# KikeM/romtime

Hardware: AMD Instinct MI355X
Metric: snapshot-DoF/s for POD build (higher is better)
Workload: dtype f64

## Files before the change

romtime_amd/csrc/tallskinny.hip:

```cpp
#include "common.h"

typedef double d2 __attribute__((ext_vector_type(2)));
typedef double d4 __attribute__((ext_vector_type(4)));

namespace {

constexpr int TS_THREADS = 256;
constexpr int TS_KS = 32;
constexpr int TS_SA = 34;

struct TsParams {
  const double* X;
  const double* T;
  double* Y;
  long N, ldx, ldt, ldy;
  int n, k;
};

template <int NT, int RB>
__global__ __launch_bounds__(TS_THREADS, RB == 2 ? (NT <= 4 ? 3 : 1) : (NT <= 4 ? 4 : 2)) void tallskinny_kernel(const TsParams p) {
  constexpr int TS_BM = 64 * RB;
  constexpr int TS_XL = TS_BM * TS_KS / 2 / TS_THREADS;
  constexpr int KP = 16 * NT;
  constexpr int TL = (TS_KS * KP / 2 + TS_THREADS - 1) / TS_THREADS;
  __shared__ __attribute__((aligned(16))) double sA[TS_BM * TS_SA];
  __shared__ __attribute__((aligned(16))) double sT[TS_KS * KP];
  const int tid = threadIdx.x, lane = tid & 63, l15 = lane & 15, l4 = lane >> 4;
  const int wid = __builtin_amdgcn_readfirstlane(tid >> 6);
  const long row0 = (long)blockIdx.x * TS_BM;
  const bool xvec = ((p.ldx & 1) == 0) && ((reinterpret_cast<size_t>(p.X) & 15) == 0);
  const bool tvec = ((p.ldt & 1) == 0) && ((reinterpret_cast<size_t>(p.T) & 15) == 0);

  d4 acc[RB][NT];
#pragma unroll
  for (int b = 0; b < RB; ++b)
#pragma unroll
    for (int j = 0; j < NT; ++j) acc[b][j] = d4{0.0, 0.0, 0.0, 0.0};

  d2 xr[TS_XL], tr[TL];
  auto fetch = [&](int c0) {
#pragma unroll
    for (int i = 0; i < TS_XL; ++i) {
      const int q = tid + TS_THREADS * i, r = q / (TS_KS / 2), c = c0 + 2 * (q % (TS_KS / 2));
      const long row = row0 + r;
      d2 v{0.0, 0.0};
      if (row < p.N) {
        const double* src = p.X + row * p.ldx + c;
        if (xvec && c + 1 < p.n) {
          v = *reinterpret_cast<const d2*>(src);
        } else {
          if (c < p.n) v.x = src[0];
          if (c + 1 < p.n) v.y = src[1];
        }
      }
      xr[i] = v;
    }
#pragma unroll
    for (int i = 0; i < TL; ++i) {
      const int q = tid + TS_THREADS * i, kk = q / (KP / 2), j = 2 * (q % (KP / 2));
      d2 v{0.0, 0.0};
      if (kk < TS_KS && c0 + kk < p.n) {
        const double* src = p.T + (long)(c0 + kk) * p.ldt + j;
        if (tvec && j + 1 < p.k) {
          v = *reinterpret_cast<const d2*>(src);
        } else {
          if (j < p.k) v.x = src[0];
          if (j + 1 < p.k) v.y = src[1];
        }
      }
      tr[i] = v;
    }
  };
  auto commit = [&]() {
#pragma unroll
    for (int i = 0; i < TS_XL; ++i) {
      const int q = tid + TS_THREADS * i, r = q / (TS_KS / 2), c = 2 * (q % (TS_KS / 2));
      *reinterpret_cast<d2*>(&sA[r * TS_SA + c]) = xr[i];
    }
#pragma unroll
    for (int i = 0; i < TL; ++i) {
      const int q = tid + TS_THREADS * i, kk = q / (KP / 2), j = 2 * (q % (KP / 2));
      if (kk < TS_KS) *reinterpret_cast<d2*>(&sT[kk * KP + j]) = tr[i];
    }
  };

  fetch(0);
  commit();
  __syncthreads();
  const double* fa = sA + (16 * wid + l15) * TS_SA + l4;
  const double* fb = sT + l4 * KP + l15;
  int c0 = 0;
  const bool fast = xvec && tvec && (row0 + TS_BM <= p.N) && (p.n % TS_KS == 0) && ((p.k & 1) == 0) &&
                    ((long)TS_BM * p.ldx * 8 < (1L << 31)) && ((long)TS_KS * p.ldt * 8 < (1L << 31));
  if (fast) {
    const char* gx = reinterpret_cast<const char*>(p.X + row0 * p.ldx + TS_KS);
    const char* gt = reinterpret_cast<const char*>(p.T + (long)TS_KS * p.ldt);
    const unsigned xoff = (unsigned)(((long)(tid / (TS_KS / 2)) * p.ldx + 2 * (tid % (TS_KS / 2))) * 8);
    const long xstep = (long)(TS_THREADS / (TS_KS / 2)) * p.ldx * 8;
    unsigned toff[TL];
    bool tuse[TL];
#pragma unroll
    for (int i = 0; i < TL; ++i) {
      const int q = tid + TS_THREADS * i, kk = q / (KP / 2), j = 2 * (q % (KP / 2));
      toff[i] = (unsigned)(((long)kk * p.ldt + j) * 8);
      tuse[i] = j + 1 < p.k;
      tr[i] = d2{0.0, 0.0};
    }
    const long tstage = (long)TS_KS * p.ldt * 8;
    for (; c0 + TS_KS < p.n; c0 += TS_KS) {
#pragma unroll
      for (int i = 0; i < TS_XL; ++i) xr[i] = *reinterpret_cast<const d2*>(gx + i * xstep + xoff);
#pragma unroll
      for (int i = 0; i < TL; ++i)
        if (tuse[i]) tr[i] = *reinterpret_cast<const d2*>(gt + toff[i]);
#pragma unroll
      for (int k4 = 0; k4 < TS_KS / 4; ++k4) {
        double bq[NT];
#pragma unroll
        for (int j = 0; j < NT; ++j) bq[j] = fb[4 * k4 * KP + 16 * j];
#pragma unroll
        for (int b = 0; b < RB; ++b) {
          const double a = fa[64 * b * TS_SA + 4 * k4];
#pragma unroll
          for (int j = 0; j < NT; ++j) acc[b][j] = __builtin_amdgcn_mfma_f64_16x16x4f64(a, bq[j], acc[b][j], 0, 0, 0);
        }
      }
      gx += TS_KS * 8;
      gt += tstage;
      __syncthreads();
      commit();
      __syncthreads();
    }
  }
  for (; c0 < p.n; c0 += TS_KS) {
    const bool more = c0 + TS_KS < p.n;
    if (more) fetch(c0 + TS_KS);
#pragma unroll
    for (int k4 = 0; k4 < TS_KS / 4; ++k4) {
      double bq[NT];
#pragma unroll
      for (int j = 0; j < NT; ++j) bq[j] = fb[4 * k4 * KP + 16 * j];
#pragma unroll
      for (int b = 0; b < RB; ++b) {
        const double a = fa[64 * b * TS_SA + 4 * k4];
#pragma unroll
        for (int j = 0; j < NT; ++j) acc[b][j] = __builtin_amdgcn_mfma_f64_16x16x4f64(a, bq[j], acc[b][j], 0, 0, 0);
      }
    }
    __syncthreads();
    if (more) commit();
    __syncthreads();
  }
#pragma unroll
  for (int b = 0; b < RB; ++b)
#pragma unroll
    for (int j = 0; j < NT; ++j)
#pragma unroll
      for (int c = 0; c < 4; ++c) {
        const long row = row0 + 64 * b + 16 * wid + l4 + 4 * c;
        const int col = 16 * j + l15;
        if (row < p.N && col < p.k) p.Y[row * p.ldy + col] = acc[b][j][c];
      }
}

}

int rt_tallskinny(rt_ctx* ctx, const double* X, int64_t ldx, const double* T, int64_t ldt, int64_t N, int64_t n,
                  int64_t k, double* Y, int64_t ldy) {
  if (k > 128 || n < 2 * TS_KS || N < 64L * ctx->num_cus) return RT_ERR_UNSUPPORTED;
  TsParams p{X, T, Y, (long)N, (long)ldx, (long)ldt, (long)ldy, (int)n, (int)k};
  const int nt = (int)((k + 15) / 16);
  const int rb = (nt <= 4 && N >= 128L * 4 * ctx->num_cus) ? 2 : 1;
  const int bm = 64 * rb;
  const unsigned grid = (unsigned)((N + bm - 1) / bm);
  if (ctx->profile) {
    if (!ctx->ev0) {
      RT_HIP_CHECK(ctx, hipEventCreate(&ctx->ev0));
      RT_HIP_CHECK(ctx, hipEventCreate(&ctx->ev1));
    }
    RT_HIP_CHECK(ctx, hipEventRecord(ctx->ev0, ctx->stream));
  }
#define TS_LAUNCH(NT_)                                                                                                  \
  if (rb == 2) hipLaunchKernelGGL((tallskinny_kernel<(NT_ <= 4 ? NT_ : 4), 2>), dim3(grid), dim3(TS_THREADS), 0, ctx->stream, p); \
  else hipLaunchKernelGGL((tallskinny_kernel<NT_, 1>), dim3(grid), dim3(TS_THREADS), 0, ctx->stream, p)
  switch (nt) {
    case 1: TS_LAUNCH(1); break;
    case 2: TS_LAUNCH(2); break;
    case 3: TS_LAUNCH(3); break;
    case 4: TS_LAUNCH(4); break;
    case 5: TS_LAUNCH(5); break;
    case 6: TS_LAUNCH(6); break;
    case 7: TS_LAUNCH(7); break;
    default: TS_LAUNCH(8); break;
  }
#undef TS_LAUNCH
  RT_HIP_CHECK(ctx, hipGetLastError());
  if (ctx->profile) {
    RT_HIP_CHECK(ctx, hipEventRecord(ctx->ev1, ctx->stream));
    ctx->ev_valid = true;
  }
  ctx->last_grid = grid; ctx->last_splits = 1; ctx->last_tile = bm * 1000 + 16 * nt;
  return RT_OK;
}
```

Before: 90.20 billion.

## Handle ragged k tail with 4x4x4 f64 MFMA instead of padding to 16

When k is not a multiple of 16, the last column group is computed with 4x4x4 f64 MFMA blocks, 4 columns each, instead of a full 16x16x4 tile. This cuts wasted matrix-core work and T loads on padded columns. Templates now split into full tiles (KF) and narrow groups (G), and the dispatch switch picks among many more instantiations. The narrow MFMA layout adds risk in how lanes map to output rows and columns, and small tails use a different instruction mix.

```diff
diff --git a/romtime_amd/csrc/tallskinny.hip b/romtime_amd/csrc/tallskinny.hip
--- a/romtime_amd/csrc/tallskinny.hip
+++ b/romtime_amd/csrc/tallskinny.hip
@@ -17,12 +17,15 @@
   int n, k;
 };
 
-template <int NT, int RB>
-__global__ __launch_bounds__(TS_THREADS, RB == 2 ? (NT <= 4 ? 3 : 1) : (NT <= 4 ? 4 : 2)) void tallskinny_kernel(const TsParams p) {
+template <int KF, int G, int RB>
+__global__ __launch_bounds__(TS_THREADS, RB == 2 ? (KF + (G > 0) <= 4 ? 3 : 1) : (KF + (G > 0) <= 4 ? 4 : 2)) void tallskinny_kernel(const TsParams p) {
+  constexpr int NT = KF + (G > 0);
   constexpr int TS_BM = 64 * RB;
   constexpr int TS_XL = TS_BM * TS_KS / 2 / TS_THREADS;
   constexpr int KP = 16 * NT;
-  constexpr int TL = (TS_KS * KP / 2 + TS_THREADS - 1) / TS_THREADS;
+  constexpr int KW = 16 * KF + 4 * G;
+  constexpr int TL = (TS_KS * KW / 2 + TS_THREADS - 1) / TS_THREADS;
+  constexpr int KF1 = KF > 0 ? KF : 1, G1 = G > 0 ? G : 1;
   __shared__ __attribute__((aligned(16))) double sA[TS_BM * TS_SA];
   __shared__ __attribute__((aligned(16))) double sT[TS_KS * KP];
   const int tid = threadIdx.x, lane = tid & 63, l15 = lane & 15, l4 = lane >> 4;
@@ -31,11 +34,15 @@
   const bool xvec = ((p.ldx & 1) == 0) && ((reinterpret_cast<size_t>(p.X) & 15) == 0);
   const bool tvec = ((p.ldt & 1) == 0) && ((reinterpret_cast<size_t>(p.T) & 15) == 0);
 
-  d4 acc[RB][NT];
-#pragma unroll
-  for (int b = 0; b < RB; ++b)
-#pragma unroll
-    for (int j = 0; j < NT; ++j) acc[b][j] = d4{0.0, 0.0, 0.0, 0.0};
+  d4 acc[RB][KF1];
+  double accg[RB][G1];
+#pragma unroll
+  for (int b = 0; b < RB; ++b) {
+#pragma unroll
+    for (int j = 0; j < KF1; ++j) acc[b][j] = d4{0.0, 0.0, 0.0, 0.0};
+#pragma unroll
+    for (int g = 0; g < G1; ++g) accg[b][g] = 0.0;
+  }
 
   d2 xr[TS_XL], tr[TL];
   auto fetch = [&](int c0) {
@@ -57,7 +64,7 @@
     }
 #pragma unroll
     for (int i = 0; i < TL; ++i) {
-      const int q = tid + TS_THREADS * i, kk = q / (KP / 2), j = 2 * (q % (KP / 2));
+      const int q = tid + TS_THREADS * i, kk = q / (KW / 2), j = 2 * (q % (KW / 2));
       d2 v{0.0, 0.0};
       if (kk < TS_KS && c0 + kk < p.n) {
         const double* src = p.T + (long)(c0 + kk) * p.ldt + j;
@@ -79,7 +86,7 @@
     }
 #pragma unroll
     for (int i = 0; i < TL; ++i) {
-      const int q = tid + TS_THREADS * i, kk = q / (KP / 2), j = 2 * (q % (KP / 2));
+      const int q = tid + TS_THREADS * i, kk = q / (KW / 2), j = 2 * (q % (KW / 2));
       if (kk < TS_KS) *reinterpret_cast<d2*>(&sT[kk * KP + j]) = tr[i];
     }
   };
@@ -89,6 +96,25 @@
   __syncthreads();
   const double* fa = sA + (16 * wid + l15) * TS_SA + l4;
   const double* fb = sT + l4 * KP + l15;
+  const double* fg = sT + l4 * KP + 16 * KF + (lane & 3);
+  auto multiply = [&]() {
+#pragma unroll
+    for (int k4 = 0; k4 < TS_KS / 4; ++k4) {
+      double bq[KF1], bg[G1];
+#pragma unroll
+      for (int j = 0; j < KF; ++j) bq[j] = fb[4 * k4 * KP + 16 * j];
+#pragma unroll
+      for (int g = 0; g < G; ++g) bg[g] = fg[4 * k4 * KP + 4 * g];
+#pragma unroll
+      for (int b = 0; b < RB; ++b) {
+        const double a = fa[64 * b * TS_SA + 4 * k4];
+#pragma unroll
+        for (int j = 0; j < KF; ++j) acc[b][j] = __builtin_amdgcn_mfma_f64_16x16x4f64(a, bq[j], acc[b][j], 0, 0, 0);
+#pragma unroll
+        for (int g = 0; g < G; ++g) accg[b][g] = __builtin_amdgcn_mfma_f64_4x4x4f64(a, bg[g], accg[b][g], 0, 0, 0);
+      }
+    }
+  };
   int c0 = 0;
   const bool fast = xvec && tvec && (row0 + TS_BM <= p.N) && (p.n % TS_KS == 0) && ((p.k & 1) == 0) &&
                     ((long)TS_BM * p.ldx * 8 < (1L << 31)) && ((long)TS_KS * p.ldt * 8 < (1L << 31));
@@ -101,9 +127,9 @@
     bool tuse[TL];
 #pragma unroll
     for (int i = 0; i < TL; ++i) {
-      const int q = tid + TS_THREADS * i, kk = q / (KP / 2), j = 2 * (q % (KP / 2));
+      const int q = tid + TS_THREADS * i, kk = q / (KW / 2), j = 2 * (q % (KW / 2));
       toff[i] = (unsigned)(((long)kk * p.ldt + j) * 8);
-      tuse[i] = j + 1 < p.k;
+      tuse[i] = kk < TS_KS && j + 1 < p.k;
       tr[i] = d2{0.0, 0.0};
     }
     const long tstage = (long)TS_KS * p.ldt * 8;
@@ -113,18 +139,7 @@
 #pragma unroll
       for (int i = 0; i < TL; ++i)
         if (tuse[i]) tr[i] = *reinterpret_cast<const d2*>(gt + toff[i]);
-#pragma unroll
-      for (int k4 = 0; k4 < TS_KS / 4; ++k4) {
-        double bq[NT];
-#pragma unroll
-        for (int j = 0; j < NT; ++j) bq[j] = fb[4 * k4 * KP + 16 * j];
-#pragma unroll
-        for (int b = 0; b < RB; ++b) {
-          const double a = fa[64 * b * TS_SA + 4 * k4];
-#pragma unroll
-          for (int j = 0; j < NT; ++j) acc[b][j] = __builtin_amdgcn_mfma_f64_16x16x4f64(a, bq[j], acc[b][j], 0, 0, 0);
-        }
-      }
+      multiply();
       gx += TS_KS * 8;
       gt += tstage;
       __syncthreads();
@@ -135,32 +150,39 @@
   for (; c0 < p.n; c0 += TS_KS) {
     const bool more = c0 + TS_KS < p.n;
     if (more) fetch(c0 + TS_KS);
-#pragma unroll
-    for (int k4 = 0; k4 < TS_KS / 4; ++k4) {
-      double bq[NT];
-#pragma unroll
-      for (int j = 0; j < NT; ++j) bq[j] = fb[4 * k4 * KP + 16 * j];
-#pragma unroll
-      for (int b = 0; b < RB; ++b) {
-        const double a = fa[64 * b * TS_SA + 4 * k4];
-#pragma unroll
-        for (int j = 0; j < NT; ++j) acc[b][j] = __builtin_amdgcn_mfma_f64_16x16x4f64(a, bq[j], acc[b][j], 0, 0, 0);
-      }
-    }
+    multiply();
     __syncthreads();
     if (more) commit();
     __syncthreads();
   }
 #pragma unroll
-  for (int b = 0; b < RB; ++b)
-#pragma unroll
-    for (int j = 0; j < NT; ++j)
+  for (int b = 0; b < RB; ++b) {
+#pragma unroll
+    for (int j = 0; j < KF; ++j)
 #pragma unroll
       for (int c = 0; c < 4; ++c) {
         const long row = row0 + 64 * b + 16 * wid + l4 + 4 * c;
         const int col = 16 * j + l15;
         if (row < p.N && col < p.k) p.Y[row * p.ldy + col] = acc[b][j][c];
       }
+#pragma unroll
+    for (int g = 0; g < G; ++g) {
+      const long row = row0 + 64 * b + 16 * wid + (l15 & 12) + l4;
+      const int col = 16 * KF + 4 * g + (lane & 3);
+      if (row < p.N && col < p.k) p.Y[row * p.ldy + col] = accg[b][g];
+    }
+  }
+}
+
+template <int KF, int G>
+void ts_launch(int rb, unsigned grid, hipStream_t stream, const TsParams& p) {
+  if constexpr (KF + (G > 0) <= 4) {
+    if (rb == 2) {
+      hipLaunchKernelGGL((tallskinny_kernel<KF, G, 2>), dim3(grid), dim3(TS_THREADS), 0, stream, p);
+      return;
+    }
+  }
+  hipLaunchKernelGGL((tallskinny_kernel<KF, G, 1>), dim3(grid), dim3(TS_THREADS), 0, stream, p);
 }
 
 }
@@ -180,20 +202,17 @@
     }
     RT_HIP_CHECK(ctx, hipEventRecord(ctx->ev0, ctx->stream));
   }
-#define TS_LAUNCH(NT_)                                                                                                  \
-  if (rb == 2) hipLaunchKernelGGL((tallskinny_kernel<(NT_ <= 4 ? NT_ : 4), 2>), dim3(grid), dim3(TS_THREADS), 0, ctx->stream, p); \
-  else hipLaunchKernelGGL((tallskinny_kernel<NT_, 1>), dim3(grid), dim3(TS_THREADS), 0, ctx->stream, p)
-  switch (nt) {
-    case 1: TS_LAUNCH(1); break;
-    case 2: TS_LAUNCH(2); break;
-    case 3: TS_LAUNCH(3); break;
-    case 4: TS_LAUNCH(4); break;
-    case 5: TS_LAUNCH(5); break;
-    case 6: TS_LAUNCH(6); break;
-    case 7: TS_LAUNCH(7); break;
-    default: TS_LAUNCH(8); break;
-  }
-#undef TS_LAUNCH
+  const int c = (int)(k % 16);
+  const int kf = (c == 0 || c >= 13) ? nt : nt - 1, g = (c == 0 || c >= 13) ? 0 : (c + 3) / 4;
+#define TS_CASE(KF_, G_) case 4 * (KF_) + (G_): ts_launch<KF_, G_>(rb, grid, ctx->stream, p); break;
+#define TS_ROW(KF_) TS_CASE(KF_, 0) TS_CASE(KF_, 1) TS_CASE(KF_, 2) TS_CASE(KF_, 3)
+  switch (4 * kf + g) {
+    TS_CASE(0, 1) TS_CASE(0, 2) TS_CASE(0, 3)
+    TS_ROW(1) TS_ROW(2) TS_ROW(3) TS_ROW(4) TS_ROW(5) TS_ROW(6) TS_ROW(7)
+    default: ts_launch<8, 0>(rb, grid, ctx->stream, p); break;
+  }
+#undef TS_ROW
+#undef TS_CASE
   RT_HIP_CHECK(ctx, hipGetLastError());
   if (ctx->profile) {
     RT_HIP_CHECK(ctx, hipEventRecord(ctx->ev1, ctx->stream));
```

Result: faster. 91.37 billion, median of 6 (+1.3%).
